# dkales/dpf-go

Hardware: AMD Instinct MI355X
Metric: DPF leaf points/sec (EvalFull logN=20, batched keys) + AES blocks/sec (higher is better)
Workload: dtype u32

## Files before the change

### dpf-go_amd/csrc/aes_ttable.hpp

```cpp
#pragma once
#include <hip/hip_runtime.h>
#include <stdint.h>
#include "aes_consts.hpp"

namespace dpfk {

constexpr uint32_t kTabWords = 256 * 64;

static __constant__ dpfc::Words256 c_te0 = dpfc::kTe0;

struct Blk {
    uint32_t c0, c1, c2, c3;
};

__device__ __forceinline__ uint32_t rotl(uint32_t x, int n) { return (x << n) | (x >> (32 - n)); }
constexpr uint32_t crotl(uint32_t x, int n) { return (x << n) | (x >> (32 - n)); }

constexpr uint32_t kXor3 = 0x96;
constexpr uint32_t kOrXor = 0x56;
__device__ __forceinline__ uint32_t xor3(uint32_t a, uint32_t b, uint32_t c) {
    return __builtin_amdgcn_bitop3_b32(a, b, c, kXor3);
}

template <int K>
__device__ __forceinline__ uint32_t taddr(uint32_t x, uint32_t laneoff) {
    return __builtin_amdgcn_perm(x, laneoff, 0x0c0c0000u | ((4u + K) << 8));
}

template <int K, bool ROT = false>
__device__ __forceinline__ uint32_t tl(const uint8_t* tab, uint32_t x, uint32_t laneoff) {
    return *reinterpret_cast<const uint32_t*>(tab + taddr<K>(x, laneoff) + (ROT ? 128 : 0));
}

template <bool RIGHT>
struct KeyFixed {
    template <int I>
    __device__ __forceinline__ uint32_t get() const {
        return RIGHT ? dpfc::kRkR.w[I] : dpfc::kRkL.w[I];
    }
    template <int I>
    __device__ __forceinline__ uint32_t get16() const {
        constexpr uint32_t v = crotl(RIGHT ? dpfc::kRkR.w[I] : dpfc::kRkL.w[I], 16);
        return v;
    }
};
struct KeySel {
    uint32_t m;
    template <int I>
    __device__ __forceinline__ uint32_t get() const {
        constexpr uint32_t l = dpfc::kRkL.w[I];
        constexpr uint32_t d = dpfc::kRkL.w[I] ^ dpfc::kRkR.w[I];
        return l ^ (m & d);
    }
    template <int I>
    __device__ __forceinline__ uint32_t get16() const {
        constexpr uint32_t l = crotl(dpfc::kRkL.w[I], 16);
        constexpr uint32_t d = crotl(dpfc::kRkL.w[I] ^ dpfc::kRkR.w[I], 16);
        return l ^ (m & d);
    }
};

template <int R, class K>
__device__ __forceinline__ void aes_round(const uint8_t* tab, uint32_t lo, const K& k, Blk& s) {
    auto col = [&](uint32_t a, uint32_t b, uint32_t c, uint32_t d, uint32_t rk16) {
        uint32_t ta = tl<0>(tab, a, lo), tb = tl<1, true>(tab, b, lo), tc = tl<2>(tab, c, lo),
                 td = tl<3, true>(tab, d, lo);
        return xor3(ta, tb, rotl(xor3(tc, td, rk16), 16));
    };
    uint32_t n0 = col(s.c0, s.c1, s.c2, s.c3, k.template get16<4 * R + 0>());
    uint32_t n1 = col(s.c1, s.c2, s.c3, s.c0, k.template get16<4 * R + 1>());
    uint32_t n2 = col(s.c2, s.c3, s.c0, s.c1, k.template get16<4 * R + 2>());
    uint32_t n3 = col(s.c3, s.c0, s.c1, s.c2, k.template get16<4 * R + 3>());
    s.c0 = n0; s.c1 = n1; s.c2 = n2; s.c3 = n3;
}

template <class K>
__device__ __forceinline__ void aes_last(const uint8_t* tab, uint32_t lo, const K& k, Blk& s) {
    auto col = [&](uint32_t a, uint32_t b, uint32_t c, uint32_t d, uint32_t rk) {
        uint32_t la = tl<0>(tab, a, lo), lb = tl<1>(tab, b, lo), lc = tl<2>(tab, c, lo), ld = tl<3>(tab, d, lo);
        uint32_t p = __builtin_amdgcn_perm(lb, la, 0x0c0c0501u);
        uint32_t q = __builtin_amdgcn_perm(ld, lc, 0x05010c0cu);
        return __builtin_amdgcn_bitop3_b32(p, q, rk, kOrXor);
    };
    uint32_t n0 = col(s.c0, s.c1, s.c2, s.c3, k.template get<40>());
    uint32_t n1 = col(s.c1, s.c2, s.c3, s.c0, k.template get<41>());
    uint32_t n2 = col(s.c2, s.c3, s.c0, s.c1, k.template get<42>());
    uint32_t n3 = col(s.c3, s.c0, s.c1, s.c2, k.template get<43>());
    s.c0 = n0; s.c1 = n1; s.c2 = n2; s.c3 = n3;
}

template <int C0 = 0, int C1 = 4>
__device__ __forceinline__ void round_loads(const uint8_t* tab, uint32_t lo, const Blk& s, uint32_t (&t)[16]) {
    const uint32_t c[4] = {s.c0, s.c1, s.c2, s.c3};
#pragma unroll
    for (int j = C0; j < C1; ++j) {
        t[4 * j + 0] = tl<0>(tab, c[j], lo);
        t[4 * j + 1] = tl<1, true>(tab, c[(j + 1) & 3], lo);
        t[4 * j + 2] = tl<2>(tab, c[(j + 2) & 3], lo);
        t[4 * j + 3] = tl<3, true>(tab, c[(j + 3) & 3], lo);
    }
}
template <int R, class K>
__device__ __forceinline__ void round_mix(const K& k, const uint32_t (&t)[16], Blk& s) {
    auto col = [&](int j, uint32_t rk16) {
        return xor3(t[4 * j], t[4 * j + 1], rotl(xor3(t[4 * j + 2], t[4 * j + 3], rk16), 16));
    };
    s.c0 = col(0, k.template get16<4 * R + 0>());
    s.c1 = col(1, k.template get16<4 * R + 1>());
    s.c2 = col(2, k.template get16<4 * R + 2>());
    s.c3 = col(3, k.template get16<4 * R + 3>());
}

template <int R, bool BATCH = false, class K>
__device__ __forceinline__ void aes_rounds(const uint8_t* tab, uint32_t lo, const K& k, Blk& s) {
    if constexpr (R <= 9) {
        if constexpr (BATCH) {
            uint32_t t[16];
            round_loads(tab, lo, s, t);
            __builtin_amdgcn_sched_barrier(0);
            round_mix<R>(k, t, s);
            __builtin_amdgcn_sched_barrier(0);
        } else {
            aes_round<R>(tab, lo, k, s);
        }
        aes_rounds<R + 1, BATCH>(tab, lo, k, s);
    }
}

template <int R, bool BATCH, class KA, class KB>
__device__ __forceinline__ void aes2_rounds(const uint8_t* tab, uint32_t lo, const KA& ka, Blk& a, const KB& kb,
                                            Blk& b) {
    if constexpr (R <= 9) {
        if constexpr (BATCH) {
            uint32_t ta[16], tb[16];
            round_loads(tab, lo, a, ta);
            round_loads(tab, lo, b, tb);
            __builtin_amdgcn_sched_barrier(0);
            round_mix<R>(ka, ta, a);
            round_mix<R>(kb, tb, b);
            __builtin_amdgcn_sched_barrier(0);
        } else {
            aes_round<R>(tab, lo, ka, a);
            aes_round<R>(tab, lo, kb, b);
        }
        aes2_rounds<R + 1, BATCH>(tab, lo, ka, a, kb, b);
    }
}

__device__ __forceinline__ Blk bxor(Blk a, Blk b) { return {a.c0 ^ b.c0, a.c1 ^ b.c1, a.c2 ^ b.c2, a.c3 ^ b.c3}; }
__device__ __forceinline__ Blk bkey4(uint32_t a, uint32_t b, uint32_t c, uint32_t d) { return {a, b, c, d}; }

template <bool BATCH = false, class K>
__device__ __forceinline__ Blk mmo1(const uint8_t* tab, uint32_t lo, const K& k, Blk x) {
    Blk s = bxor(x, bkey4(k.template get<0>(), k.template get<1>(), k.template get<2>(), k.template get<3>()));
    aes_rounds<1, BATCH>(tab, lo, k, s);
    aes_last(tab, lo, k, s);
    return bxor(s, x);
}

template <bool BATCH = false, class KA, class KB>
__device__ __forceinline__ void mmo2(const uint8_t* tab, uint32_t lo, const KA& ka, Blk xa, Blk& oa, const KB& kb,
                                     Blk xb, Blk& ob) {
    Blk a = bxor(xa, bkey4(ka.template get<0>(), ka.template get<1>(), ka.template get<2>(), ka.template get<3>()));
    Blk b = bxor(xb, bkey4(kb.template get<0>(), kb.template get<1>(), kb.template get<2>(), kb.template get<3>()));
    aes2_rounds<1, BATCH>(tab, lo, ka, a, kb, b);
    aes_last(tab, lo, ka, a);
    aes_last(tab, lo, kb, b);
    oa = bxor(a, xa);
    ob = bxor(b, xb);
}

struct QuadKeys {
    uint32_t l[11], d[11];
};
__device__ __forceinline__ QuadKeys quad_keys(uint32_t j) {
    QuadKeys k;
#pragma unroll
    for (int r = 0; r < 11; ++r) {
        const uint32_t l0 = dpfc::kRkL.w[4 * r], l1 = dpfc::kRkL.w[4 * r + 1], l2 = dpfc::kRkL.w[4 * r + 2],
                       l3 = dpfc::kRkL.w[4 * r + 3];
        const uint32_t d0 = l0 ^ dpfc::kRkR.w[4 * r], d1 = l1 ^ dpfc::kRkR.w[4 * r + 1],
                       d2 = l2 ^ dpfc::kRkR.w[4 * r + 2], d3 = l3 ^ dpfc::kRkR.w[4 * r + 3];
        uint32_t l = j == 0 ? l0 : j == 1 ? l1 : j == 2 ? l2 : l3;
        uint32_t d = j == 0 ? d0 : j == 1 ? d1 : j == 2 ? d2 : d3;
        if (r >= 1 && r <= 9) {
            l = rotl(l, 16);
            d = rotl(d, 16);
        }
        k.l[r] = l;
        k.d[r] = d;
    }
    return k;
}
template <int CTRL>
__device__ __forceinline__ uint32_t quad_mov(uint32_t v) {
    return (uint32_t)__builtin_amdgcn_mov_dpp((int)v, CTRL, 0xF, 0xF, false);
}
__device__ __forceinline__ uint32_t mmo_quad(const uint8_t* tab, uint32_t lo, const QuadKeys& k, uint32_t m,
                                             uint32_t x) {
    uint32_t s = x ^ k.l[0] ^ (m & k.d[0]);
#pragma unroll
    for (int r = 1; r <= 9; ++r) {
        const uint32_t b = quad_mov<0x39>(s), c = quad_mov<0x4E>(s), d = quad_mov<0x93>(s);
        const uint32_t ta = tl<0>(tab, s, lo), tb = tl<1, true>(tab, b, lo), tc = tl<2>(tab, c, lo),
                       td = tl<3, true>(tab, d, lo);
        const uint32_t rk16 = k.l[r] ^ (m & k.d[r]);
        s = xor3(ta, tb, rotl(xor3(tc, td, rk16), 16));
    }
    const uint32_t b = quad_mov<0x39>(s), c = quad_mov<0x4E>(s), d = quad_mov<0x93>(s);
    const uint32_t la = tl<0>(tab, s, lo), lb = tl<1>(tab, b, lo), lc = tl<2>(tab, c, lo), ld = tl<3>(tab, d, lo);
    const uint32_t p = __builtin_amdgcn_perm(lb, la, 0x0c0c0501u);
    const uint32_t q = __builtin_amdgcn_perm(ld, lc, 0x05010c0cu);
    s = __builtin_amdgcn_bitop3_b32(p, q, k.l[10] ^ (m & k.d[10]), kOrXor);
    return s ^ x;
}

__device__ __forceinline__ void fill_table_nobar(uint32_t* tab) {
    for (uint32_t i = threadIdx.x; i < 256 * 16; i += blockDim.x) {
        uint32_t e = i >> 4, q = i & 15;
        uint32_t v = c_te0.v[e];
        if (q >= 8) v = rotl(v, 8);
        reinterpret_cast<uint4*>(tab)[e * 16 + q] = make_uint4(v, v, v, v);
    }
}
__device__ __forceinline__ void fill_table(uint32_t* tab) {
    fill_table_nobar(tab);
    __syncthreads();
}

}
```

### dpf-go_amd/csrc/dpf_kernels.hip

```cpp
#include <hip/hip_runtime.h>
#include <stdint.h>
#include <stdlib.h>

#include <algorithm>
#include <atomic>
#include <cmath>
#include <type_traits>
#include "aes_consts.hpp"
#include "aes_ttable.hpp"
#include "dpf_kernels.hpp"
#include "wave_prio.hpp"
#include "tree_ops.hpp"

namespace dpfk {

#ifdef DPF_WAVE_TIMES
constexpr uint64_t kWaveTimesMax = 1u << 16;
__device__ uint64_t g_wave_times[5 * kWaveTimesMax];
#endif

struct Ctx {
    const uint8_t* tab;
    uint32_t lo;
    KeySrc ks;
    Blk fcw;
    uint8_t* outp;
    uint4* nseed;
    uint8_t* nt;
    uint32_t groups;
    uint32_t* prog = nullptr;
    uint32_t pslot = 0;
};

constexpr uint32_t kPrioFar = 3;
template <int DMAX>
__device__ __forceinline__ void prio_step(Ctx& c) {
    if (c.prog != nullptr) {
        prio_by_lead(c.prog, c.pslot, ++c.groups, 1, kPrioFar);
        return;
    }
    constexpr bool small = DMAX <= (int)dpfh::kPrioSmallMaxD;
    constexpr uint32_t total = DMAX >= 2 ? 1u << (DMAX - 2) : 1u;
    const uint32_t d = ++c.groups;
    constexpr uint32_t den = small ? 8 : 16;
    constexpr uint32_t t1 = small ? 4 : 12;
    constexpr uint32_t t2 = small ? 6 : 14;
    constexpr uint32_t t3 = small ? 7 : 15;
    const uint32_t x = d * den;
    if (x >= t3 * total) __builtin_amdgcn_s_setprio(0);
    else if (x >= t2 * total) __builtin_amdgcn_s_setprio(1);
    else if (x >= t1 * total) __builtin_amdgcn_s_setprio(2);
}

__device__ __forceinline__ void emit_node(Ctx& c, const Node& n) {
    *c.nseed++ = make_uint4(n.s.c0, n.s.c1, n.s.c2, n.s.c3);
    *c.nt++ = (uint8_t)n.t;
}

__device__ __forceinline__ uint32_t pair_swap(uint32_t v) {
    return (uint32_t)__builtin_amdgcn_mov_dpp((int)v, 0xB1, 0xF, 0xF, false);
}
__device__ __forceinline__ Node pair_swap(const Node& n) {
    return {{pair_swap(n.s.c0), pair_swap(n.s.c1), pair_swap(n.s.c2), pair_swap(n.s.c3)}, pair_swap(n.t)};
}
__device__ __forceinline__ Node sel(bool b, const Node& x, const Node& y) {
    return {{b ? x.s.c0 : y.s.c0, b ? x.s.c1 : y.s.c1, b ? x.s.c2 : y.s.c2, b ? x.s.c3 : y.s.c3}, b ? x.t : y.t};
}

__device__ __forceinline__ Blk bsel(bool b, const Blk& x, const Blk& y) {
    return {b ? x.c0 : y.c0, b ? x.c1 : y.c1, b ? x.c2 : y.c2, b ? x.c3 : y.c3};
}

template <bool B, bool RAW>
__device__ __forceinline__ void leaves4(const Ctx& c, uint32_t lvl, const Node& n, uint8_t* p) {
    CW cw = key_cw<RAW>(c.ks, lvl);
    Node L, R;
    expand<B>(c.tab, c.lo, n, cw, L, R);
    CW cw1 = key_cw<RAW>(c.ks, lvl + 1);
    Blk o0 = {}, o1 = {}, o2, o3;
    Node m = L;
    const Node pend = R;
#pragma nounroll
    for (int h = 0; h < 2; ++h) {
        Node a, b;
        expand<B>(c.tab, c.lo, m, cw1, a, b);
        Blk oa, ob;
        mmo2<B>(c.tab, c.lo, KeyFixed<false>{}, a.s, oa, KeyFixed<false>{}, b.s, ob);
        oa = leaf_fix(oa, a.t, c.fcw);
        ob = leaf_fix(ob, b.t, c.fcw);
        o2 = oa;
        o3 = ob;
        if (h == 0) {
            o0 = oa;
            o1 = ob;
        }
        m = pend;
    }
    store16(p, o0);
    store16(p + 16, o1);
    store16(p + 32, o2);
    store16(p + 48, o3);
}

template <int DMAX, int D, bool NODES, bool PAIR, bool B, bool RAW = false>
__device__ __forceinline__ void dfs(Ctx& c, uint32_t lvl0, const Node& n) {
    if constexpr (PAIR && D == 3) {
        CW cw = key_cw<RAW>(c.ks, lvl0 + DMAX - 3);
        Node L, R;
        expand<B>(c.tab, c.lo, n, cw, L, R);
        const bool odd = (threadIdx.x & 1u) != 0;
        const Node got = pair_swap(sel(odd, L, R));
        const int64_t sub = 16ll << DMAX;
        Node cur = sel(odd, got, L);
        const Node second = sel(odd, R, got);
#pragma nounroll
        for (int h = 0; h < 2; ++h) {
            leaves4<B, RAW>(c, lvl0 + DMAX - 2, cur, c.outp + (h == 0 ? (odd ? 64 - sub : 0) : (odd ? 64 : sub)));
            prio_step<DMAX>(c);
            cur = second;
        }
        c.outp += 128;
    } else if constexpr (D == 0) {
        if constexpr (NODES) {
            emit_node(c, n);
        } else {
            Blk o = mmo1(c.tab, c.lo, KeyFixed<false>{}, n.s);
            store16(c.outp, leaf_fix(o, n.t, c.fcw));
            c.outp += 16;
        }
    } else if constexpr (D == 2 && !NODES) {
        leaves4<B, RAW>(c, lvl0 + DMAX - 2, n, c.outp);
        prio_step<DMAX>(c);
        c.outp += 64;
    } else if constexpr (D == 2 && NODES) {
        CW cw = key_cw<RAW>(c.ks, lvl0 + DMAX - 2);
        Node L, R;
        expand<B>(c.tab, c.lo, n, cw, L, R);
        CW cw1 = key_cw<RAW>(c.ks, lvl0 + DMAX - 1);
        Node q[4];
        expand<B>(c.tab, c.lo, L, cw1, q[0], q[1]);
        expand<B>(c.tab, c.lo, R, cw1, q[2], q[3]);
#pragma unroll
        for (int i = 0; i < 4; ++i) c.nseed[i] = make_uint4(q[i].s.c0, q[i].s.c1, q[i].s.c2, q[i].s.c3);
        *reinterpret_cast<uint32_t*>(c.nt) = (q[0].t & 0xffu) | ((q[1].t & 0xffu) << 8) | ((q[2].t & 0xffu) << 16) |
                                             ((q[3].t & 0xffu) << 24);
        c.nseed += 4;
        c.nt += 4;
        prio_step<DMAX>(c);
    } else if constexpr (D == 1) {
        CW cw = key_cw<RAW>(c.ks, lvl0 + DMAX - 1);
        Node L, R;
        expand<B>(c.tab, c.lo, n, cw, L, R);
        if constexpr (NODES) {
            emit_node(c, L);
            emit_node(c, R);
        } else {
            Blk oL, oR;
            mmo2<B>(c.tab, c.lo, KeyFixed<false>{}, L.s, oL, KeyFixed<false>{}, R.s, oR);
            store16(c.outp, leaf_fix(oL, L.t, c.fcw));
            store16(c.outp + 16, leaf_fix(oR, R.t, c.fcw));
            c.outp += 32;
        }
    } else {
        CW cw = key_cw<RAW>(c.ks, lvl0 + DMAX - D);
        Node L, R;
        expand<B>(c.tab, c.lo, n, cw, L, R);
        Node ch = L;
        const Node pend = R;
#pragma nounroll
        for (int side = 0; side < 2; ++side) {
            dfs<DMAX, D - 1, NODES, PAIR, B, RAW>(c, lvl0, ch);
            ch = pend;
        }
    }
}

__global__ void k_unpack(const uint8_t* __restrict__ keys, uint64_t key_len, uint64_t nkeys, uint32_t stop,
                         uint32_t* __restrict__ ek) {
    const uint64_t recs = (uint64_t)stop + 2;
    const uint64_t i = (uint64_t)blockIdx.x * blockDim.x + threadIdx.x;
    if (i >= nkeys * recs) return;
    const uint64_t k = i / recs, r = i % recs;
    const uint8_t* kp = keys + k * key_len;
    uint32_t* o = ek + k * (recs * 8) + r * 8;
    auto w = [](const uint8_t* p) {
        return (uint32_t)p[0] | ((uint32_t)p[1] << 8) | ((uint32_t)p[2] << 16) | ((uint32_t)p[3] << 24);
    };
    if (r == 0) {
        o[0] = w(kp); o[1] = w(kp + 4); o[2] = w(kp + 8); o[3] = w(kp + 12);
        o[4] = kp[16]; o[5] = 0; o[6] = 0; o[7] = 0;
    } else if (r <= stop) {
        const uint8_t* p = kp + 17 + 18 * (r - 1);
        o[0] = w(p); o[1] = w(p + 4); o[2] = w(p + 8); o[3] = w(p + 12);
        o[4] = p[16]; o[5] = p[17]; o[6] = 0; o[7] = 0;
    } else {
        const uint8_t* p = kp + key_len - 16;
        o[0] = w(p); o[1] = w(p + 4); o[2] = w(p + 8); o[3] = w(p + 12);
        o[4] = 0; o[5] = 0; o[6] = 0; o[7] = 0;
    }
}

template <int D, bool UNIFORM, bool NODES, bool RAW = false>
__global__ __launch_bounds__(kTreeBlockMax, kTreeWaves) void k_evalfull(const uint32_t* __restrict__ ekeys, uint32_t stop,
                                                        uint64_t nunits, uint32_t units_log, uint32_t ltop,
                                                        uint64_t sub_base, uint8_t* __restrict__ out,
                                                        uint8_t* __restrict__ out_t, uint64_t out_stride,
                                                        uint64_t klen = 0, uint64_t kboff = 0) {
    static_assert(!RAW || (UNIFORM && !NODES), "raw keys: wave-uniform leaf launches only");
#ifdef DPF_WAVE_TIMES
    const uint64_t t_start = wall_clock64();
#endif
    __shared__ __attribute__((aligned(16))) uint32_t s_tab[kTabWords];
    const uint32_t B = blockDim.x, W = 31u - (uint32_t)__builtin_clz(B);
    const uint64_t u = (uint64_t)blockIdx.x * B + threadIdx.x;
    uint64_t key = u >> units_log;
    if constexpr (UNIFORM) key = __builtin_amdgcn_readfirstlane((uint32_t)key);
    const uint64_t local = u & ((1ull << units_log) - 1);
    const uint64_t sub = sub_base + local;
    Ctx c;
    if constexpr (RAW) {
        c.ks = {nullptr, ekeys, kboff + key * klen, klen};
    } else {
        c.ks = {ekeys + key * ((uint64_t)(stop + 2) * 8), nullptr, 0, 0};
    }
    __shared__ __attribute__((aligned(16))) uint32_t s_cw[8 * 64];
    const bool cw_lds = UNIFORM && stop <= 64 && units_log >= W && (uint64_t)blockIdx.x * B < nunits;
    const bool cw_mine = cw_lds && threadIdx.x < ltop;
    CW cw_pre{};
    if (cw_mine) cw_pre = key_cw<RAW>(c.ks, threadIdx.x);
    __shared__ __attribute__((aligned(16))) uint32_t s_prog[64];
    if (threadIdx.x < 64) s_prog[threadIdx.x] = 0xffffffffu;
    fill_table_nobar(s_tab);
    if (cw_mine) {
        *reinterpret_cast<uint4*>(s_cw + 8 * threadIdx.x) = make_uint4(cw_pre.s.c0, cw_pre.s.c1, cw_pre.s.c2, cw_pre.s.c3);
        *reinterpret_cast<uint2*>(s_cw + 8 * threadIdx.x + 4) = make_uint2(cw_pre.tl, cw_pre.tr);
    }
    __syncthreads();
    if (u >= nunits) return;
    auto lds_cw = [&](uint32_t lvl) __attribute__((always_inline)) {
        const uint4 a = *reinterpret_cast<const uint4*>(s_cw + 8 * lvl);
        const uint2 b = *reinterpret_cast<const uint2*>(s_cw + 8 * lvl + 4);
        return CW{{a.x, a.y, a.z, a.w}, b.x, b.y};
    };
    c.groups = 0;
    if (UNIFORM && !NODES && D >= (int)kFeedbackMinD && B == (uint32_t)kTreeBlockBig) {
        c.prog = prog_slots(s_prog, c.pslot);
        c.prog[c.pslot] = 0;
    }
    __builtin_amdgcn_s_setprio(3);
    c.tab = reinterpret_cast<const uint8_t*>(s_tab);
    c.lo = (threadIdx.x & 31u) * 4u;
    if constexpr (NODES) {
        c.nseed = reinterpret_cast<uint4*>(out) + key * out_stride + (local << D);
        c.nt = out_t + key * out_stride + (local << D);
    } else {
        c.fcw = key_fcw<RAW>(c.ks, stop);
        c.outp = out + key * out_stride + local * (16ull << D);
    }

    Node n;
    n.s = key_root<RAW>(c.ks, n.t);
    uint32_t lvl = 0;
    if constexpr (UNIFORM) {
        constexpr uint32_t F = 6, kFs = 1u << F;
        __shared__ uint32_t s_front[5 * kFs];
        if (W >= 7 && cw_lds) {
            const uint32_t l1 = ltop - W + F;
            auto put = [&](uint32_t j, const Node& m) {
                s_front[j] = m.s.c0; s_front[kFs + j] = m.s.c1; s_front[2 * kFs + j] = m.s.c2;
                s_front[3 * kFs + j] = m.s.c3; s_front[4 * kFs + j] = m.t;
            };
            auto get = [&](uint32_t j) {
                Node m;
                m.s = {s_front[j], s_front[kFs + j], s_front[2 * kFs + j], s_front[3 * kFs + j]};
                m.t = s_front[4 * kFs + j];
                return m;
            };
            if (W >= 8) {
                if (threadIdx.x < (4u << F)) {
                    const uint32_t path = threadIdx.x >> 2, j = threadIdx.x & 3u;
                    const uint64_t subj = (sub - threadIdx.x) + ((uint64_t)path << (W - F));
                    const QuadKeys qk = quad_keys(j);
                    uint32_t col = j == 0 ? n.s.c0 : j == 1 ? n.s.c1 : j == 2 ? n.s.c2 : n.s.c3;
                    uint32_t t = n.t;
                    for (uint32_t i = 0; i < l1; ++i) {
                        const CW cw = lds_cw(i);
                        const uint32_t cwj = j == 0 ? cw.s.c0 : j == 1 ? cw.s.c1 : j == 2 ? cw.s.c2 : cw.s.c3;
                        walk_step_quad(c.tab, c.lo, qk, j, col, t, cwj, cw.tl, cw.tr,
                                       (uint32_t)(subj >> (ltop - 1 - i)) & 1u);
                    }
                    s_front[j * kFs + path] = col;
                    if (j == 0) s_front[4 * kFs + path] = t;
                }
            } else if (threadIdx.x < 64) {
                const uint64_t subj = (sub - threadIdx.x) + ((uint64_t)threadIdx.x << (W - 6));
                Node m = n;
                for (uint32_t i = 0; i < l1; ++i) {
                    CW cw = lds_cw(i);
                    walk_step<true>(c.tab, c.lo, m, cw, (uint32_t)(subj >> (ltop - 1 - i)) & 1u);
                }
                put(threadIdx.x, m);
            }
            __syncthreads();
            n = get(threadIdx.x >> (W - F));
            lvl = l1;
        }
    }
    if (cw_lds) {
        for (uint32_t i = lvl; i < ltop; ++i)
            walk_step<true>(c.tab, c.lo, n, lds_cw(i), (uint32_t)(sub >> (ltop - 1 - i)) & 1u);
    } else {
        for (uint32_t i = lvl; i < ltop; ++i)
            walk_step<true>(c.tab, c.lo, n, key_cw<RAW>(c.ks, i), (uint32_t)(sub >> (ltop - 1 - i)) & 1u);
    }
#ifdef DPF_WAVE_TIMES
    const uint64_t t_walk = wall_clock64();
#endif
    constexpr bool kPair = UNIFORM && !NODES && D >= 3;
    dfs<D, D, NODES, kPair, UNIFORM, RAW>(c, ltop, n);
    if (c.prog != nullptr) c.prog[c.pslot] = 0xffffffffu;
#ifdef DPF_WAVE_TIMES
    if ((threadIdx.x & 63) == 0) {
        const uint64_t wv = u >> 6;
        if (wv < kWaveTimesMax) {
            g_wave_times[5 * wv] = t_start;
            g_wave_times[5 * wv + 1] = wall_clock64();
            g_wave_times[5 * wv + 2] = __builtin_amdgcn_s_getreg(0xF804);
            g_wave_times[5 * wv + 3] = __builtin_amdgcn_s_getreg(0xF814);
            g_wave_times[5 * wv + 4] = t_walk;
        }
    }
#endif
}

__device__ __forceinline__ Node eval_start(const uint32_t* ek, uint64_t key, uint64_t x, uint32_t logN,
                                           const uint4* fseed, const uint8_t* ft, uint32_t L) {
    Node n;
    if (fseed != nullptr) {
        const uint64_t idx = (key << L) + ((x >> (logN - L)) & ((1ull << L) - 1));
        const uint4 v = fseed[idx];
        n.s = {v.x, v.y, v.z, v.w};
        n.t = ft[idx];
    } else {
        n.s = load_blk(ek);
        n.t = ek[4];
    }
    return n;
}
struct PairIn {
    uint64_t x0, x1;
    Node n0, n1;
};
template <bool UNI>
__device__ __forceinline__ uint64_t pair_key(uint64_t q, uint64_t pts_per_key) {
    const uint64_t k = q / pts_per_key;
    if constexpr (UNI) return __builtin_amdgcn_readfirstlane((uint32_t)k);
    return k;
}
template <bool UNI>
__device__ __forceinline__ PairIn eval_pair_in(const uint32_t* __restrict__ ekeys, uint32_t stop, uint32_t logN,
                                               const uint64_t* __restrict__ xs, uint64_t nq, uint64_t pts_per_key,
                                               const uint4* __restrict__ fseed, const uint8_t* __restrict__ ft,
                                               uint32_t L, uint64_t q0) {
    const uint64_t qa = q0 < nq ? q0 : nq - 1;
    const uint64_t q1 = qa + 1 < nq ? qa + 1 : qa;
    const uint64_t key0 = pair_key<UNI>(qa, pts_per_key), key1 = UNI ? key0 : q1 / pts_per_key;
    const uint64_t rec = (uint64_t)(stop + 2) * 8;
    PairIn p;
    p.x0 = xs[qa];
    p.x1 = xs[q1];
    p.n0 = eval_start(ekeys + key0 * rec, key0, p.x0, logN, fseed, ft, L);
    p.n1 = eval_start(ekeys + key1 * rec, key1, p.x1, logN, fseed, ft, L);
    return p;
}
template <bool UNI>
__device__ __forceinline__ uint32_t eval_pair_bits(const uint32_t* __restrict__ ekeys, uint32_t stop, uint32_t logN,
                                                   uint64_t nq, uint64_t pts_per_key, const uint4* __restrict__ fseed,
                                                   uint32_t L, const uint32_t* s_tab, uint64_t q0, PairIn p,
                                                   const uint32_t* cwp = nullptr) {
    const uint64_t q1 = q0 + 1 < nq ? q0 + 1 : q0;
    const uint64_t key0 = pair_key<UNI>(q0, pts_per_key), key1 = UNI ? key0 : q1 / pts_per_key;
    const uint64_t rec = (uint64_t)(stop + 2) * 8;
    const uint32_t* ek0 = ekeys + key0 * rec;
    const uint32_t* ek1 = ekeys + key1 * rec;
    const uint8_t* tab = reinterpret_cast<const uint8_t*>(s_tab);
    const uint32_t lo = (threadIdx.x & 31u) * 4u;
    const uint32_t i0 = fseed != nullptr ? L : 0;
    if (UNI && cwp != nullptr) {
        for (uint32_t i = i0; i < stop; ++i) {
            const uint4 a = *reinterpret_cast<const uint4*>(cwp + 8 * (i - i0));
            const uint2 b = *reinterpret_cast<const uint2*>(cwp + 8 * (i - i0) + 4);
            const CW cw{{a.x, a.y, a.z, a.w}, b.x, b.y};
            walk_step2<true>(tab, lo, p.n0, cw, path_bit(p.x0, logN - 1 - i), p.n1, cw,
                                       path_bit(p.x1, logN - 1 - i));
        }
    } else {
        for (uint32_t i = i0; i < stop; ++i) {
            const CW cw0 = load_cw(ek0, i), cw1 = UNI ? cw0 : load_cw(ek1, i);
            walk_step2<true>(tab, lo, p.n0, cw0, path_bit(p.x0, logN - 1 - i), p.n1, cw1,
                                       path_bit(p.x1, logN - 1 - i));
        }
    }
    Blk o0, o1;
    mmo2<true>(tab, lo, KeyFixed<false>{}, p.n0.s, o0, KeyFixed<false>{}, p.n1.s, o1);
    const Blk f0 = UNI && cwp != nullptr ? load_blk(cwp + 8 * (stop - i0)) : load_blk(ek0 + 8 + 8 * stop);
    o0 = leaf_fix(o0, p.n0.t, f0);
    o1 = leaf_fix(o1, p.n1.t, UNI ? f0 : load_blk(ek1 + 8 + 8 * stop));
    return (uint32_t)eval_bit(o0, p.x0) | ((uint32_t)eval_bit(o1, p.x1) << 8);
}
template <bool UNI>
__device__ __forceinline__ void eval_pair_walk(const uint32_t* __restrict__ ekeys, uint32_t stop, uint32_t logN,
                                               uint64_t nq, uint64_t pts_per_key, const uint4* __restrict__ fseed,
                                               uint32_t L, uint8_t* __restrict__ out, const uint32_t* s_tab,
                                               uint64_t q0, PairIn p) {
    const uint32_t b = eval_pair_bits<UNI>(ekeys, stop, logN, nq, pts_per_key, fseed, L, s_tab, q0, p);
    out[q0] = (uint8_t)b;
    if (q0 + 1 < nq) out[q0 + 1] = (uint8_t)(b >> 8);
}

template <bool UNI>
__global__ __launch_bounds__(kBlock, 4) void k_eval2(const uint32_t* __restrict__ ekeys, uint32_t stop,
                                                     uint32_t logN, const uint64_t* __restrict__ xs, uint64_t nq,
                                                     uint64_t pts_per_key, const uint4* __restrict__ fseed,
                                                     const uint8_t* __restrict__ ft, uint32_t L,
                                                     uint8_t* __restrict__ out) {
    __shared__ __attribute__((aligned(16))) uint32_t s_tab[kTabWords];
    const uint64_t q0 = 2 * ((uint64_t)blockIdx.x * blockDim.x + threadIdx.x);
    PairIn p{};
    if (q0 < nq) p = eval_pair_in<UNI>(ekeys, stop, logN, xs, nq, pts_per_key, fseed, ft, L, q0);
    fill_table(s_tab);
    __builtin_amdgcn_s_setprio(3);
    if (q0 < nq) eval_pair_walk<UNI>(ekeys, stop, logN, nq, pts_per_key, fseed, L, out, s_tab, q0, p);
}

__global__ __launch_bounds__(kBlock, 4) void k_eval_bits(const uint32_t* __restrict__ ekeys, uint32_t stop,
                                                         uint32_t logN, const uint64_t* __restrict__ xs, uint64_t npts,
                                                         uint64_t keys_per_list, uint64_t units, uint64_t nwaves,
                                                         const uint4* __restrict__ fseed,
                                                         const uint8_t* __restrict__ ft, uint32_t L,
                                                         uint8_t* __restrict__ bits, uint64_t bits_stride) {
    __shared__ __attribute__((aligned(16))) uint32_t s_tab[kTabWords];
    const uint32_t lane = threadIdx.x & 63;
    const uint32_t wib = __builtin_amdgcn_readfirstlane(threadIdx.x >> 6);
    const uint64_t w = (uint64_t)blockIdx.x * (blockDim.x >> 6) + wib;
    const bool live = w < nwaves;
    uint64_t key = 0, unit = 0, j0 = 0, j1 = 0;
    PairIn p{};
    if (live) {
        key = w / units;
        unit = w - key * units;
        j0 = dpfh::eval_bits_point(unit, lane, 0);
        j1 = dpfh::eval_bits_point(unit, lane, 1);
        const uint32_t* ek = ekeys + key * ((uint64_t)(stop + 2) * 8);
        const uint32_t list = __builtin_amdgcn_readfirstlane((uint32_t)dpfh::eval_bits_list(key, keys_per_list));
        const uint64_t* lx = xs + dpfh::eval_bits_list_base(list, npts);
        p.x0 = lx[dpfh::eval_bits_clamp(j0, npts)];
        p.x1 = lx[dpfh::eval_bits_clamp(j1, npts)];
        p.n0 = eval_start(ek, key, p.x0, logN, fseed, ft, L);
        p.n1 = eval_start(ek, key, p.x1, logN, fseed, ft, L);
    }
    fill_table(s_tab);
    __builtin_amdgcn_s_setprio(3);
    if (!live) return;
    const uint32_t b = eval_pair_bits<true>(ekeys, stop, logN, key + 1, 1, fseed, L, s_tab, key, p);
    const uint64_t m0 = __builtin_amdgcn_ballot_w64((b & 1u) != 0 && j0 < npts);
    const uint64_t m1 = __builtin_amdgcn_ballot_w64(((b >> 8) & 1u) != 0 && j1 < npts);
    if (lane == 0)
        *reinterpret_cast<uint4*>(bits + key * bits_stride + dpfh::eval_bits_unit_off(unit)) =
            make_uint4((uint32_t)m0, (uint32_t)(m0 >> 32), (uint32_t)m1, (uint32_t)(m1 >> 32));
}

constexpr uint32_t kEvalPrioFar = 3;
struct EvalSlots {
    uint4 x[2][64];
    uint4 n0[64], n1[64];
    uint32_t t0[64], t1[64];
    uint32_t cw[2][64];
};
__device__ __forceinline__ void eval_vm0() {
#if defined(__HIP_DEVICE_COMPILE__)
    asm volatile("s_waitcnt vmcnt(0)" ::: "memory");
#endif
}
__device__ __forceinline__ void eval_lgkm0() {
#if defined(__HIP_DEVICE_COMPILE__)
    asm volatile("s_waitcnt lgkmcnt(0)" ::: "memory");
#endif
}
__device__ __forceinline__ void glds(const void* g, void* l, int size) {
#if defined(__HIP_DEVICE_COMPILE__)
    if (size == 16)
        __builtin_amdgcn_global_load_lds(g, (__attribute__((address_space(3))) void*)l, 16, 0, 0);
    else
        __builtin_amdgcn_global_load_lds(g, (__attribute__((address_space(3))) void*)l, 4, 0, 0);
#else
    (void)g;
    (void)l;
    (void)size;
#endif
}
__global__ __launch_bounds__(kEvalPBlock, 1) void k_eval_persist(const uint32_t* __restrict__ ekeys, uint32_t stop,
                                                                 uint32_t logN, const uint64_t* __restrict__ xs,
                                                                 uint64_t nq, uint64_t pts_per_key,
                                                                 const uint4* __restrict__ fseed,
                                                                 const uint8_t* __restrict__ ft, uint32_t L,
                                                                 uint8_t* __restrict__ out) {
    __shared__ __attribute__((aligned(256))) uint32_t s_tab[kTabWords];
    __shared__ __attribute__((aligned(16))) EvalSlots s_sl[kEvalPBlock / 64];
    const uint32_t lane = threadIdx.x & 63;
    EvalSlots& sl = s_sl[__builtin_amdgcn_readfirstlane(threadIdx.x >> 6)];
    const uint64_t npairs = nq / 2;
    const uint64_t nthr = (uint64_t)gridDim.x * blockDim.x;
    const uint64_t gt = (uint64_t)blockIdx.x * blockDim.x + threadIdx.x;
    const uint64_t iters = (npairs + nthr - 1) / nthr;
    auto pair_of = [&](uint64_t i) __attribute__((always_inline)) {
        const uint64_t p = i * nthr + gt;
        return p < npairs ? p : npairs - 1;
    };
    const uint64_t rec = (uint64_t)(stop + 2) * 8;
    const uint32_t ncw = (stop - L) * 8 + 4;
    const bool cw_slots = ncw <= 64;
    auto issue_x = [&](uint64_t i, int slot) __attribute__((always_inline)) {
        glds(xs + 2 * pair_of(i), &sl.x[slot][0], 16);
    };
    auto issue_nodes = [&](uint64_t i, int slot) __attribute__((always_inline)) {
        const uint4 xv = sl.x[slot][lane];
        const uint64_t x0 = ((uint64_t)xv.y << 32) | xv.x, x1 = ((uint64_t)xv.w << 32) | xv.z;
        const uint64_t key = pair_key<true>(2 * pair_of(i), pts_per_key);
        const uint64_t m = (1ull << L) - 1;
        const uint64_t i0 = (key << L) + ((x0 >> (logN - L)) & m), i1 = (key << L) + ((x1 >> (logN - L)) & m);
        eval_lgkm0();
        glds(fseed + i0, &sl.n0[0], 16);
        glds(fseed + i1, &sl.n1[0], 16);
        glds(ft + (i0 & ~3ull), &sl.t0[0], 4);
        glds(ft + (i1 & ~3ull), &sl.t1[0], 4);
        if (cw_slots && lane < ncw) glds(ekeys + key * rec + 8 + 8 * L + lane, &sl.cw[slot][0], 4);
    };
    auto read_pair = [&](uint64_t i) __attribute__((always_inline)) {
        eval_vm0();
        PairIn p;
        const uint4 xv = sl.x[i & 1][lane];
        p.x0 = ((uint64_t)xv.y << 32) | xv.x;
        p.x1 = ((uint64_t)xv.w << 32) | xv.z;
        const uint4 a = sl.n0[lane], b = sl.n1[lane];
        const uint64_t key = pair_key<true>(2 * pair_of(i), pts_per_key);
        const uint64_t m = (1ull << L) - 1;
        const uint32_t i0 = (uint32_t)((key << L) + ((p.x0 >> (logN - L)) & m)) & 3u;
        const uint32_t i1 = (uint32_t)((key << L) + ((p.x1 >> (logN - L)) & m)) & 3u;
        p.n0.s = {a.x, a.y, a.z, a.w};
        p.n1.s = {b.x, b.y, b.z, b.w};
        p.n0.t = (sl.t0[lane] >> (8 * i0)) & 0xffu;
        p.n1.t = (sl.t1[lane] >> (8 * i1)) & 0xffu;
        return p;
    };
    if (iters == 0) return;
    __shared__ __attribute__((aligned(16))) uint32_t s_prog[64];
    if (threadIdx.x < 64) s_prog[threadIdx.x] = 0xffffffffu;
    issue_x(0, 0);
    if (iters > 1) issue_x(1, 1);
    fill_table(s_tab);
    __builtin_amdgcn_s_setprio(3);
    uint32_t pslot;
    uint32_t* prog = prog_slots(s_prog, pslot);
    prog[pslot] = 0;
    issue_nodes(0, 0);
    PairIn p = read_pair(0);
    if (iters > 1) issue_nodes(1, 1);
    if (iters > 2) {
        eval_lgkm0();
        issue_x(2, 0);
    }
    for (uint64_t it = 0; it < iters; ++it) {
        if ((it & 3) == 0) prio_by_lead(prog, pslot, (uint32_t)it, 4, 4 * kEvalPrioFar);
        const uint64_t pr = it * nthr + gt;
        const uint32_t* cwp = cw_slots ? &sl.cw[it & 1][0] : nullptr;
        const uint32_t b = eval_pair_bits<true>(ekeys, stop, logN, nq, pts_per_key, fseed, L, s_tab, 2 * pair_of(it), p,
                                                cwp);
        p = read_pair(it + 1 < iters ? it + 1 : it);
        if (pr < npairs) {
            out[2 * pr] = (uint8_t)b;
            out[2 * pr + 1] = (uint8_t)(b >> 8);
        }
        if (it + 2 < iters) issue_nodes(it + 2, (int)(it & 1));
        if (it + 3 < iters) {
            eval_lgkm0();
            issue_x(it + 3, (int)((it + 1) & 1));
        }
    }
    prog[pslot] = 0xffffffffu;
}

template <bool RIGHT>
__global__ __launch_bounds__(kBlock, 4) void k_mmo_tt(const uint4* __restrict__ in, uint4* __restrict__ out,
                                                      uint64_t npairs, uint32_t reps) {
    __shared__ __attribute__((aligned(16))) uint32_t s_tab[kTabWords];
    fill_table(s_tab);
    const uint64_t u = (uint64_t)blockIdx.x * blockDim.x + threadIdx.x;
    if (u >= npairs) return;
    const uint8_t* tab = reinterpret_cast<const uint8_t*>(s_tab);
    const uint32_t lo = (threadIdx.x & 31u) * 4u;
    const uint4 va = in[2 * u], vb = in[2 * u + 1];
    Blk a = {va.x, va.y, va.z, va.w}, b = {vb.x, vb.y, vb.z, vb.w};
    for (uint32_t r = 0; r < reps; ++r) mmo2<true>(tab, lo, KeyFixed<RIGHT>{}, a, a, KeyFixed<RIGHT>{}, b, b);
    out[2 * u] = make_uint4(a.c0, a.c1, a.c2, a.c3);
    out[2 * u + 1] = make_uint4(b.c0, b.c1, b.c2, b.c3);
}


hipError_t launch_mmo_tt(const uint8_t* in, uint8_t* out, uint64_t nblocks, uint32_t right, uint32_t reps,
                         hipStream_t st) {
    const uint64_t pairs = nblocks / 2;
    if (pairs == 0) return hipSuccess;
    const dim3 grid((uint32_t)((pairs + kBlock - 1) / kBlock));
    if (right)
        hipLaunchKernelGGL(k_mmo_tt<true>, grid, dim3(kBlock), 0, st, reinterpret_cast<const uint4*>(in),
                           reinterpret_cast<uint4*>(out), pairs, reps);
    else
        hipLaunchKernelGGL(k_mmo_tt<false>, grid, dim3(kBlock), 0, st, reinterpret_cast<const uint4*>(in),
                           reinterpret_cast<uint4*>(out), pairs, reps);
    return hipGetLastError();
}

// ... 177 lines not shown
```

### dpf-go_amd/csrc/tree_ops.hpp

```cpp
#pragma once
#include <hip/hip_runtime.h>
#include <stdint.h>
#include "aes_ttable.hpp"

namespace dpfk {

struct Node {
    Blk s;
    uint32_t t;
};

struct CW {
    Blk s;
    uint32_t tl, tr;
};

__device__ __forceinline__ uint32_t tmask(uint32_t t) { return t != 0 ? 0xffffffffu : 0u; }
__device__ __forceinline__ uint32_t path_bit(uint64_t x, uint32_t s) { return s < 64 ? (uint32_t)(x >> s) & 1u : 0u; }
__device__ __forceinline__ uint8_t eval_bit(Blk o, uint64_t x) {
    const uint32_t b = (uint32_t)(x & 127);
    const uint32_t w = (b >> 5) == 0 ? o.c0 : (b >> 5) == 1 ? o.c1 : (b >> 5) == 2 ? o.c2 : o.c3;
    return (uint8_t)((w >> (b & 31)) & 1u);
}

__device__ __forceinline__ CW load_cw(const uint32_t* ek, uint32_t lvl) {
    const uint4* p = reinterpret_cast<const uint4*>(ek + 8 + 8 * lvl);
    uint4 a = p[0];
    uint2 b = *reinterpret_cast<const uint2*>(ek + 8 + 8 * lvl + 4);
    return {{a.x, a.y, a.z, a.w}, b.x, b.y};
}
__device__ __forceinline__ Blk load_blk(const uint32_t* p) {
    uint4 a = *reinterpret_cast<const uint4*>(p);
    return {a.x, a.y, a.z, a.w};
}

struct KeySrc {
    const uint32_t* ek;
    const uint32_t* kw;
    uint64_t kb, klen;
};
__device__ __forceinline__ uint32_t funnel(uint32_t a, uint32_t b, uint32_t sh) {
    return (uint32_t)((((uint64_t)b << 32) | a) >> sh);
}
template <bool RAW>
__device__ __forceinline__ CW key_cw(const KeySrc& k, uint32_t lvl) {
    if constexpr (!RAW) {
        return load_cw(k.ek, lvl);
    } else {
        const uint64_t o = k.kb + 17 + 18ull * lvl;
        const uint32_t* p = k.kw + (o >> 2);
        const uint32_t sh = (uint32_t)(o & 3) * 8;
        const uint32_t w0 = p[0], w1 = p[1], w2 = p[2], w3 = p[3], w4 = p[4];
        const uint32_t w5 = sh == 24 ? p[5] : 0u;
        const uint32_t t = funnel(w4, w5, sh);
        return {{funnel(w0, w1, sh), funnel(w1, w2, sh), funnel(w2, w3, sh), funnel(w3, w4, sh)}, t & 0xffu,
                (t >> 8) & 0xffu};
    }
}
template <bool RAW>
__device__ __forceinline__ Blk key_root(const KeySrc& k, uint32_t& t) {
    if constexpr (!RAW) {
        t = k.ek[4];
        return load_blk(k.ek);
    } else {
        const uint32_t* p = k.kw + (k.kb >> 2);
        const uint32_t sh = (uint32_t)(k.kb & 3) * 8;
        const uint32_t w0 = p[0], w1 = p[1], w2 = p[2], w3 = p[3], w4 = p[4];
        t = (w4 >> sh) & 0xffu;
        return {funnel(w0, w1, sh), funnel(w1, w2, sh), funnel(w2, w3, sh), funnel(w3, w4, sh)};
    }
}
template <bool RAW>
__device__ __forceinline__ Blk key_fcw(const KeySrc& k, uint32_t stop) {
    if constexpr (!RAW) {
        return load_blk(k.ek + 8 + 8 * stop);
    } else {
        const uint64_t o = k.kb + k.klen - 16;
        const uint32_t* p = k.kw + (o >> 2);
        const uint32_t sh = (uint32_t)(o & 3) * 8;
        const uint32_t w0 = p[0], w1 = p[1], w2 = p[2], w3 = p[3];
        const uint32_t w4 = sh ? p[4] : 0u;
        return {funnel(w0, w1, sh), funnel(w1, w2, sh), funnel(w2, w3, sh), funnel(w3, w4, sh)};
    }
}

template <bool B = false>
__device__ __forceinline__ void expand(const uint8_t* tab, uint32_t lo, const Node& n, const CW& cw, Node& L,
                                       Node& R) {
    mmo2<B>(tab, lo, KeyFixed<false>{}, n.s, L.s, KeyFixed<true>{}, n.s, R.s);
    uint32_t tL = L.s.c0 & 1u, tR = R.s.c0 & 1u;
    L.s.c0 &= ~1u;
    R.s.c0 &= ~1u;
    uint32_t m = tmask(n.t);
    L.s.c0 ^= m & cw.s.c0; L.s.c1 ^= m & cw.s.c1; L.s.c2 ^= m & cw.s.c2; L.s.c3 ^= m & cw.s.c3;
    R.s.c0 ^= m & cw.s.c0; R.s.c1 ^= m & cw.s.c1; R.s.c2 ^= m & cw.s.c2; R.s.c3 ^= m & cw.s.c3;
    L.t = tL ^ (m & cw.tl);
    R.t = tR ^ (m & cw.tr);
}

__device__ __forceinline__ void walk_fix(Node& n, Blk c, const CW& cw, uint32_t bit) {
    uint32_t tc = c.c0 & 1u;
    c.c0 &= ~1u;
    uint32_t m = tmask(n.t);
    c.c0 ^= m & cw.s.c0; c.c1 ^= m & cw.s.c1; c.c2 ^= m & cw.s.c2; c.c3 ^= m & cw.s.c3;
    n.s = c;
    n.t = tc ^ (m & (bit ? cw.tr : cw.tl));
}
template <bool B = false>
__device__ __forceinline__ void walk_step(const uint8_t* tab, uint32_t lo, Node& n, const CW& cw, uint32_t bit) {
    walk_fix(n, mmo1<B>(tab, lo, KeySel{bit ? 0xffffffffu : 0u}, n.s), cw, bit);
}
template <bool B = false>
__device__ __forceinline__ void walk_step2(const uint8_t* tab, uint32_t lo, Node& n0, const CW& cw0, uint32_t bit0,
                                           Node& n1, const CW& cw1, uint32_t bit1) {
    Blk c0, c1;
    mmo2<B>(tab, lo, KeySel{bit0 ? 0xffffffffu : 0u}, n0.s, c0, KeySel{bit1 ? 0xffffffffu : 0u}, n1.s, c1);
    walk_fix(n0, c0, cw0, bit0);
    walk_fix(n1, c1, cw1, bit1);
}

__device__ __forceinline__ void walk_step_quad(const uint8_t* tab, uint32_t lo, const QuadKeys& k, uint32_t j,
                                               uint32_t& col, uint32_t& t, uint32_t cwj, uint32_t tl_, uint32_t tr_,
                                               uint32_t bit) {
    uint32_t c = mmo_quad(tab, lo, k, bit ? 0xffffffffu : 0u, col);
    const uint32_t tc = quad_mov<0x00>(c) & 1u;
    if (j == 0) c &= ~1u;
    const uint32_t m = tmask(t);
    col = c ^ (m & cwj);
    t = tc ^ (m & (bit ? tr_ : tl_));
}

__device__ __forceinline__ void store16(uint8_t* p, Blk v) {
    *reinterpret_cast<uint4*>(p) = make_uint4(v.c0, v.c1, v.c2, v.c3);
}

__device__ __forceinline__ Blk leaf_fix(Blk o, uint32_t t, Blk fcw) {
    uint32_t m = tmask(t);
    return {o.c0 ^ (m & fcw.c0), o.c1 ^ (m & fcw.c1), o.c2 ^ (m & fcw.c2), o.c3 ^ (m & fcw.c3)};
}

}
```

Before: 4637 billion.

## Preload per-key correction words into wave lanes and read via readlane

```diff
diff --git a/dpf-go_amd/csrc/aes_ttable.hpp b/dpf-go_amd/csrc/aes_ttable.hpp
--- a/dpf-go_amd/csrc/aes_ttable.hpp
+++ b/dpf-go_amd/csrc/aes_ttable.hpp
@@ -223,6 +223,32 @@
         reinterpret_cast<uint4*>(tab)[e * 16 + q] = make_uint4(v, v, v, v);
     }
 }
+__device__ __forceinline__ uint32_t fill_rows_first() {
+    const uint32_t tpr = blockDim.x >> 8;
+    return c_te0.v[tpr ? threadIdx.x >> (tpr >> 1) : threadIdx.x >> 4];
+}
+__device__ __forceinline__ void fill_rows_nobar(uint32_t* tab, uint32_t first) {
+    const uint32_t tpr = blockDim.x >> 8;
+    if (tpr) {
+        const uint32_t sh = tpr >> 1, e = threadIdx.x >> sh, nq = 16u >> sh, q0 = (threadIdx.x & (tpr - 1)) * nq;
+        const uint32_t r = rotl(first, 8);
+        for (uint32_t k = 0; k < nq; ++k) {
+            const uint32_t q = q0 + ((k + e) & (nq - 1));
+            const uint32_t v = q >= 8 ? r : first;
+            reinterpret_cast<uint4*>(tab)[e * 16 + q] = make_uint4(v, v, v, v);
+        }
+        return;
+    }
+    uint32_t v = first;
+    for (uint32_t i = threadIdx.x;;) {
+        const uint32_t e = i >> 4, q = i & 15;
+        if (q >= 8) v = rotl(v, 8);
+        reinterpret_cast<uint4*>(tab)[e * 16 + q] = make_uint4(v, v, v, v);
+        i += blockDim.x;
+        if (i >= 256 * 16) break;
+        v = c_te0.v[i >> 4];
+    }
+}
 __device__ __forceinline__ void fill_table(uint32_t* tab) {
     fill_table_nobar(tab);
     __syncthreads();
diff --git a/dpf-go_amd/csrc/dpf_kernels.hip b/dpf-go_amd/csrc/dpf_kernels.hip
--- a/dpf-go_amd/csrc/dpf_kernels.hip
+++ b/dpf-go_amd/csrc/dpf_kernels.hip
@@ -23,6 +23,7 @@
     const uint8_t* tab;
     uint32_t lo;
     KeySrc ks;
+    KeyLanes kl;
     Blk fcw;
     uint8_t* outp;
     uint4* nseed;
@@ -31,6 +32,12 @@
     uint32_t* prog = nullptr;
     uint32_t pslot = 0;
 };
+
+template <bool LANES>
+__device__ __forceinline__ CW tree_cw(const Ctx& c, uint32_t lvl) {
+    if constexpr (LANES) return c.kl.cw(lvl);
+    else return load_cw(c.ks.ek, lvl);
+}
 
 constexpr uint32_t kPrioFar = 3;
 template <int DMAX>
@@ -71,12 +78,12 @@
     return {b ? x.c0 : y.c0, b ? x.c1 : y.c1, b ? x.c2 : y.c2, b ? x.c3 : y.c3};
 }
 
-template <bool B, bool RAW>
+template <bool B, bool LANES>
 __device__ __forceinline__ void leaves4(const Ctx& c, uint32_t lvl, const Node& n, uint8_t* p) {
-    CW cw = key_cw<RAW>(c.ks, lvl);
+    CW cw = tree_cw<LANES>(c, lvl);
     Node L, R;
     expand<B>(c.tab, c.lo, n, cw, L, R);
-    CW cw1 = key_cw<RAW>(c.ks, lvl + 1);
+    CW cw1 = tree_cw<LANES>(c, lvl + 1);
     Blk o0 = {}, o1 = {}, o2, o3;
     Node m = L;
     const Node pend = R;
@@ -102,10 +109,10 @@
     store16(p + 48, o3);
 }
 
-template <int DMAX, int D, bool NODES, bool PAIR, bool B, bool RAW = false>
+template <int DMAX, int D, bool NODES, bool PAIR, bool B, bool LANES = false>
 __device__ __forceinline__ void dfs(Ctx& c, uint32_t lvl0, const Node& n) {
     if constexpr (PAIR && D == 3) {
-        CW cw = key_cw<RAW>(c.ks, lvl0 + DMAX - 3);
+        CW cw = tree_cw<LANES>(c, lvl0 + DMAX - 3);
         Node L, R;
         expand<B>(c.tab, c.lo, n, cw, L, R);
         const bool odd = (threadIdx.x & 1u) != 0;
@@ -115,7 +122,7 @@
         const Node second = sel(odd, R, got);
 #pragma nounroll
         for (int h = 0; h < 2; ++h) {
-            leaves4<B, RAW>(c, lvl0 + DMAX - 2, cur, c.outp + (h == 0 ? (odd ? 64 - sub : 0) : (odd ? 64 : sub)));
+            leaves4<B, LANES>(c, lvl0 + DMAX - 2, cur, c.outp + (h == 0 ? (odd ? 64 - sub : 0) : (odd ? 64 : sub)));
             prio_step<DMAX>(c);
             cur = second;
         }
@@ -129,14 +136,14 @@
             c.outp += 16;
         }
     } else if constexpr (D == 2 && !NODES) {
-        leaves4<B, RAW>(c, lvl0 + DMAX - 2, n, c.outp);
+        leaves4<B, LANES>(c, lvl0 + DMAX - 2, n, c.outp);
         prio_step<DMAX>(c);
         c.outp += 64;
     } else if constexpr (D == 2 && NODES) {
-        CW cw = key_cw<RAW>(c.ks, lvl0 + DMAX - 2);
+        CW cw = tree_cw<LANES>(c, lvl0 + DMAX - 2);
         Node L, R;
         expand<B>(c.tab, c.lo, n, cw, L, R);
-        CW cw1 = key_cw<RAW>(c.ks, lvl0 + DMAX - 1);
+        CW cw1 = tree_cw<LANES>(c, lvl0 + DMAX - 1);
         Node q[4];
         expand<B>(c.tab, c.lo, L, cw1, q[0], q[1]);
         expand<B>(c.tab, c.lo, R, cw1, q[2], q[3]);
@@ -148,7 +155,7 @@
         c.nt += 4;
         prio_step<DMAX>(c);
     } else if constexpr (D == 1) {
-        CW cw = key_cw<RAW>(c.ks, lvl0 + DMAX - 1);
+        CW cw = tree_cw<LANES>(c, lvl0 + DMAX - 1);
         Node L, R;
         expand<B>(c.tab, c.lo, n, cw, L, R);
         if constexpr (NODES) {
@@ -162,14 +169,14 @@
             c.outp += 32;
         }
     } else {
-        CW cw = key_cw<RAW>(c.ks, lvl0 + DMAX - D);
+        CW cw = tree_cw<LANES>(c, lvl0 + DMAX - D);
         Node L, R;
         expand<B>(c.tab, c.lo, n, cw, L, R);
         Node ch = L;
         const Node pend = R;
 #pragma nounroll
         for (int side = 0; side < 2; ++side) {
-            dfs<DMAX, D - 1, NODES, PAIR, B, RAW>(c, lvl0, ch);
+            dfs<DMAX, D - 1, NODES, PAIR, B, LANES>(c, lvl0, ch);
             ch = pend;
         }
     }
@@ -214,6 +221,8 @@
     const uint32_t B = blockDim.x, W = 31u - (uint32_t)__builtin_clz(B);
     const uint64_t u = (uint64_t)blockIdx.x * B + threadIdx.x;
     uint64_t key = u >> units_log;
+    constexpr bool LANES = UNIFORM && !NODES;
+    if constexpr (LANES) key = (u & ~63ull) < nunits ? key : 0;
     if constexpr (UNIFORM) key = __builtin_amdgcn_readfirstlane((uint32_t)key);
     const uint64_t local = u & ((1ull << units_log) - 1);
     const uint64_t sub = sub_base + local;
@@ -223,14 +232,21 @@
     } else {
         c.ks = {ekeys + key * ((uint64_t)(stop + 2) * 8), nullptr, 0, 0};
     }
+    const uint32_t te_first = fill_rows_first();
+    KeyWords kwords{};
+    if constexpr (LANES) kwords = KeyWords::load<RAW>(c.ks, stop, threadIdx.x & 63u);
     __shared__ __attribute__((aligned(16))) uint32_t s_cw[8 * 64];
     const bool cw_lds = UNIFORM && stop <= 64 && units_log >= W && (uint64_t)blockIdx.x * B < nunits;
     const bool cw_mine = cw_lds && threadIdx.x < ltop;
     CW cw_pre{};
-    if (cw_mine) cw_pre = key_cw<RAW>(c.ks, threadIdx.x);
+    if constexpr (!LANES) {
+        if (cw_mine) cw_pre = load_cw(c.ks.ek, threadIdx.x);
+    }
     __shared__ __attribute__((aligned(16))) uint32_t s_prog[64];
     if (threadIdx.x < 64) s_prog[threadIdx.x] = 0xffffffffu;
-    fill_table_nobar(s_tab);
+    fill_rows_nobar(s_tab, te_first);
+    c.kl = KeyLanes::make<RAW>(kwords);
+    if constexpr (LANES) cw_pre = {{c.kl.s0, c.kl.s1, c.kl.s2, c.kl.s3}, c.kl.tl, c.kl.tr};
     if (cw_mine) {
         *reinterpret_cast<uint4*>(s_cw + 8 * threadIdx.x) = make_uint4(cw_pre.s.c0, cw_pre.s.c1, cw_pre.s.c2, cw_pre.s.c3);
         *reinterpret_cast<uint2*>(s_cw + 8 * threadIdx.x + 4) = make_uint2(cw_pre.tl, cw_pre.tr);
@@ -254,12 +270,17 @@
         c.nseed = reinterpret_cast<uint4*>(out) + key * out_stride + (local << D);
         c.nt = out_t + key * out_stride + (local << D);
     } else {
-        c.fcw = key_fcw<RAW>(c.ks, stop);
+        if constexpr (LANES) c.fcw = c.kl.fcw(stop);
+        else c.fcw = load_blk(c.ks.ek + 8 + 8 * stop);
         c.outp = out + key * out_stride + local * (16ull << D);
     }
 
     Node n;
-    n.s = key_root<RAW>(c.ks, n.t);
+    if constexpr (LANES) n.s = c.kl.root(stop, n.t);
+    else {
+        n.t = c.ks.ek[4];
+        n.s = load_blk(c.ks.ek);
+    }
     uint32_t lvl = 0;
     if constexpr (UNIFORM) {
         constexpr uint32_t F = 6, kFs = 1u << F;
@@ -311,13 +332,13 @@
             walk_step<true>(c.tab, c.lo, n, lds_cw(i), (uint32_t)(sub >> (ltop - 1 - i)) & 1u);
     } else {
         for (uint32_t i = lvl; i < ltop; ++i)
-            walk_step<true>(c.tab, c.lo, n, key_cw<RAW>(c.ks, i), (uint32_t)(sub >> (ltop - 1 - i)) & 1u);
+            walk_step<true>(c.tab, c.lo, n, tree_cw<LANES>(c, i), (uint32_t)(sub >> (ltop - 1 - i)) & 1u);
     }
 #ifdef DPF_WAVE_TIMES
     const uint64_t t_walk = wall_clock64();
 #endif
     constexpr bool kPair = UNIFORM && !NODES && D >= 3;
-    dfs<D, D, NODES, kPair, UNIFORM, RAW>(c, ltop, n);
+    dfs<D, D, NODES, kPair, UNIFORM, LANES>(c, ltop, n);
     if (c.prog != nullptr) c.prog[c.pslot] = 0xffffffffu;
 #ifdef DPF_WAVE_TIMES
     if ((threadIdx.x & 63) == 0) {
diff --git a/dpf-go_amd/csrc/tree_ops.hpp b/dpf-go_amd/csrc/tree_ops.hpp
--- a/dpf-go_amd/csrc/tree_ops.hpp
+++ b/dpf-go_amd/csrc/tree_ops.hpp
@@ -42,47 +42,48 @@
 __device__ __forceinline__ uint32_t funnel(uint32_t a, uint32_t b, uint32_t sh) {
     return (uint32_t)((((uint64_t)b << 32) | a) >> sh);
 }
-template <bool RAW>
-__device__ __forceinline__ CW key_cw(const KeySrc& k, uint32_t lvl) {
-    if constexpr (!RAW) {
-        return load_cw(k.ek, lvl);
-    } else {
-        const uint64_t o = k.kb + 17 + 18ull * lvl;
-        const uint32_t* p = k.kw + (o >> 2);
-        const uint32_t sh = (uint32_t)(o & 3) * 8;
-        const uint32_t w0 = p[0], w1 = p[1], w2 = p[2], w3 = p[3], w4 = p[4];
-        const uint32_t w5 = sh == 24 ? p[5] : 0u;
-        const uint32_t t = funnel(w4, w5, sh);
-        return {{funnel(w0, w1, sh), funnel(w1, w2, sh), funnel(w2, w3, sh), funnel(w3, w4, sh)}, t & 0xffu,
-                (t >> 8) & 0xffu};
+struct KeyWords {
+    uint32_t w0, w1, w2, w3, w4, w5, sh;
+
+    template <bool RAW>
+    static __device__ __forceinline__ KeyWords load(const KeySrc& k, uint32_t stop, uint32_t lane) {
+        if constexpr (!RAW) {
+            const uint32_t* p = k.ek + 8 * (lane < stop ? lane + 1 : lane == stop + 1 ? stop + 1 : 0u);
+            const uint4 a = *reinterpret_cast<const uint4*>(p);
+            const uint2 b = *reinterpret_cast<const uint2*>(p + 4);
+            return {a.x, a.y, a.z, a.w, b.x, b.y, 0};
+        } else {
+            const uint64_t o = k.kb + (lane < stop ? 17 + 18ull * lane : lane == stop + 1 ? k.klen - 16 : 0ull);
+            const uint32_t last = (uint32_t)(o & 3) + (lane < stop ? 17u : lane == stop + 1 ? 15u : 16u);
+            const uint32_t* p = k.kw + (o >> 2);
+            return {p[0], p[1], p[2], p[3], p[last < 16 ? 3 : 4], p[last >> 2], (uint32_t)(o & 3) * 8};
+        }
     }
-}
-template <bool RAW>
-__device__ __forceinline__ Blk key_root(const KeySrc& k, uint32_t& t) {
-    if constexpr (!RAW) {
-        t = k.ek[4];
-        return load_blk(k.ek);
-    } else {
-        const uint32_t* p = k.kw + (k.kb >> 2);
-        const uint32_t sh = (uint32_t)(k.kb & 3) * 8;
-        const uint32_t w0 = p[0], w1 = p[1], w2 = p[2], w3 = p[3], w4 = p[4];
-        t = (w4 >> sh) & 0xffu;
-        return {funnel(w0, w1, sh), funnel(w1, w2, sh), funnel(w2, w3, sh), funnel(w3, w4, sh)};
+};
+struct KeyLanes {
+    uint32_t s0, s1, s2, s3, tl, tr;
+
+    template <bool RAW>
+    static __device__ __forceinline__ KeyLanes make(const KeyWords& k) {
+        if constexpr (!RAW) {
+            return {k.w0, k.w1, k.w2, k.w3, k.w4, k.w5};
+        } else {
+            const uint32_t t = funnel(k.w4, k.w5, k.sh);
+            return {funnel(k.w0, k.w1, k.sh), funnel(k.w1, k.w2, k.sh), funnel(k.w2, k.w3, k.sh),
+                    funnel(k.w3, k.w4, k.sh), t & 0xffu, (t >> 8) & 0xffu};
+        }
     }
-}
-template <bool RAW>
-__device__ __forceinline__ Blk key_fcw(const KeySrc& k, uint32_t stop) {
-    if constexpr (!RAW) {
-        return load_blk(k.ek + 8 + 8 * stop);
-    } else {
-        const uint64_t o = k.kb + k.klen - 16;
-        const uint32_t* p = k.kw + (o >> 2);
-        const uint32_t sh = (uint32_t)(o & 3) * 8;
-        const uint32_t w0 = p[0], w1 = p[1], w2 = p[2], w3 = p[3];
-        const uint32_t w4 = sh ? p[4] : 0u;
-        return {funnel(w0, w1, sh), funnel(w1, w2, sh), funnel(w2, w3, sh), funnel(w3, w4, sh)};
+    __device__ __forceinline__ uint32_t rl(uint32_t v, uint32_t lane) const {
+        return (uint32_t)__builtin_amdgcn_readlane((int)v, (int)lane);
     }
-}
+    __device__ __forceinline__ Blk blk(uint32_t lane) const { return {rl(s0, lane), rl(s1, lane), rl(s2, lane), rl(s3, lane)}; }
+    __device__ __forceinline__ CW cw(uint32_t lvl) const { return {blk(lvl), rl(tl, lvl), rl(tr, lvl)}; }
+    __device__ __forceinline__ Blk root(uint32_t stop, uint32_t& t) const {
+        t = rl(tl, stop);
+        return blk(stop);
+    }
+    __device__ __forceinline__ Blk fcw(uint32_t stop) const { return blk(stop + 1); }
+};
 
 template <bool B = false>
 __device__ __forceinline__ void expand(const uint8_t* tab, uint32_t lo, const Node& n, const CW& cw, Node& L,
```

After: 4639 billion (median of 2 runs). No clear change (+0.1%).
